# ImIntheMiddle/VATL4Pose-WACV2024

Hardware: AMD Instinct MI355X
Metric: frames/sec pose-infer+uncertainty, 256x192 17-kp (higher is better)
Workload: dtype f32; 1 GPU; SimpleBaseline-R50 256x192 inference + decode + local-peak + THC-L1, 1024-frame synthetic video per GPU; frames_per_gpu=1024, batch=1024, tracks=4, parallelism=frame-sharded x1

## Files before the change

include/vatl_hip.h:

```cpp
#ifndef VATL_HIP_H
#define VATL_HIP_H

#include <stdint.h>

#ifdef __cplusplus
extern "C" {
#endif

#define VATL_VERSION 100
#define VATL_EINVAL  (-1)
#define VATL_ELAUNCH (-2)

int         vatl_version(void);
const char* vatl_last_error(void);

int vatl_flop_meter_begin(void);
int vatl_flop_meter_end(double* direct_flops, double* winograd_flops, int64_t* direct_launches, int64_t* winograd_launches);
#define VATL_ROUTE_NAMES "igemm,igemm_bnbwd,igemm_dma,persistent_1x1,streamk,rows_1x1,bottleneck_chain,stem_pool,halo_3x3," \
                         "winograd,winograd_2h,winograd_bnbwd,winograd_persist,winograd_c32,wgrad,winograd_wgrad,winograd_wgrad_2h," \
                         "winograd_wgrad_table,winograd_f4,winograd_f4_bnbwd,gemm1x1_ring"
int vatl_flop_meter_routes(int64_t* counts, int n);


int vatl_nchw_to_nhwc(const float* src, float* dst, int N, int C, int H, int W, int Cpad, void* stream);
int vatl_nhwc_to_nchw(const float* src, float* dst, int N, int C, int H, int W, void* stream);

int vatl_pack_conv_weight(const float* w_oihw, float* w_packed, int Cout, int Cin, int R, int S,
                          int CoutPad, int Spad, int CinPad, void* stream);
int vatl_pack_deconv4x4s2_weight(const float* w_iohw, float* w_packed, int Cin, int Cout, int CoutPad, void* stream);
int64_t vatl_stem_pool_weight_floats(void);
int vatl_pack_stem_pool_weight(const float* w_oihw, float* packed, void* stream);
int vatl_stem_pool_supported(int H, int W);
int vatl_stem7x7s2_pool_fwd(const float* x_nchw, const float* w_packed, const float* scale, const float* bias, float* y_nhwc,
                            int N, int H, int W, void* stream);
int64_t vatl_stem3_weight_floats(void);
int vatl_pack_stem3_weight(const float* w_oihw, float* packed, void* stream);
int vatl_stem3x3s2_fwd(const float* x_nchw, const float* w_packed, const float* scale, const float* bias, float* y_nhwc,
                       int N, int H, int W, void* stream);

int vatl_bn_fold(const float* gamma, const float* beta, const float* mean, const float* var, const float* conv_bias,
                 float eps, float* scale, float* bias, int C, void* stream);


int vatl_pack_conv1x1_dual_weight(const float* w1, const float* scale1, const float* bias1, const float* w2, const float* scale2,
                                  const float* bias2, float* out, float* bias, int Cout, int C1, int C2, int CoutPad, void* stream);
int vatl_conv1x1_dual_fwd(const float* a, const float* x, const float* w, const float* bias, float* y, int N, int Ho, int Wo,
                          int C1, int H2, int W2, int C2, int stride2, int Cout, int CoutPad, int relu, void* stream);

int64_t vatl_winograd_c32_weight_floats(void);
int vatl_pack_winograd_c32_weight(const float* w, float* u, void* stream);
int vatl_conv3x3_winograd_c32_supported(int N, int H, int W, int Cin, int Cout);
int vatl_conv3x3_winograd_c32_fwd(const float* x, const float* u, const float* scale, const float* bias, const float* residual, float* y, int N, int H, int W,
                                  int relu, void* stream);

int64_t vatl_winograd_f4_weight_floats(int Cout, int Cin);
int vatl_pack_winograd_f4_weight(const float* w, float* u, int Cout, int Cin, int data_gradient, void* stream);
int vatl_conv3x3_winograd_f4_supported(int N, int H, int W, int Cin, int Cout);
int vatl_conv3x3_winograd_f4_fwd(const float* x, const float* u, const float* scale, const float* bias, const float* residual, float* y, int N, int H, int W,
                                 int Cin, int Cout, int relu, void* stream);
int64_t vatl_winograd_f4_stats_row_blocks(int64_t N, int H, int W);
int vatl_conv3x3_winograd_f4_fwd_stats(const float* x, const float* u, float* y, double* stats, int64_t* row_blocks_used, int N, int H, int W, int Cin, int Cout,
                                       void* stream);
int vatl_conv3x3_winograd_f4_fwd_bnbwd(const float* x, const float* u, const float* residual, float* y, int N, int H, int W, int Cin, int Cout, const float* bn_z,
                                       const float* bn_mask_y, const float* bn_scale, const float* bn_bias, const float* bn_mean, const float* bn_invstd,
                                       double* stats, int64_t* row_blocks_used, void* stream);

int vatl_conv1x1_rows_supported(int K1, int K2, int N, int64_t M);
int vatl_conv1x1_rows_fwd(const float* a, const float* x2, const float* w, const float* scale, const float* bias, const float* residual, float* y,
                          int64_t M, int K1, int K2, int N, int relu, void* stream);

int vatl_bottleneck_chain_supported(int Cmid, int Cout, int Cnext, int64_t M);
int vatl_bottleneck_chain_fwd(const float* a, const float* w3, const float* scale3, const float* bias3, const float* skip, float* t,
                              const float* w1, const float* scale1, const float* bias1, float* y1, int64_t M, int Cmid, int Cout,
                              int Cnext, void* stream);

int vatl_tune_set(int knob, int value);
int vatl_set_splitk_workspace(float* workspace, int64_t floats);
int vatl_set_splitk_workspace_thread(float* workspace, int64_t floats);
int64_t vatl_streamk_workspace_bytes(void);
int vatl_set_streamk_workspace_thread(void* workspace, int64_t bytes);
int vatl_conv_cout_pad(int Cout);
int vatl_conv2d_fwd(const float* x, const float* w, const float* scale, const float* bias, const float* residual,
                    float* y, int N, int H, int W, int Cin, int Cout, int CoutPad, int R, int S, int stride, int pad,
                    int relu, int out_nchw, void* stream);

int vatl_deconv4x4s2_fwd(const float* x, const float* w, const float* scale, const float* bias, float* y,
                         int N, int H, int W, int Cin, int Cout, int CoutPad, int relu, void* stream);

int vatl_maxpool3x3s2_fwd(const float* x, float* y, int N, int H, int W, int C, void* stream);
int vatl_gap_fwd(const float* x, float* y, int N, int HW, int C, void* stream);

int vatl_pixelshuffle2_fwd(const float* x, float* y, int N, int H, int W, int C, void* stream);
int vatl_se_scale_add_relu(const float* x, const float* gate, const float* residual, float* y, int N, int HW, int C, void* stream);
int vatl_fuse_upsample_add(const float* base, const float* z0, int shift0, const float* z1, int shift1, const float* z2, int shift2,
                           float* y, int N, int H, int W, int C, int relu, void* stream);
int vatl_upsample_nearest_bwd(const float* dy, const float* yact_or_null, float* dz, int N, int H, int W, int C, int shift, void* stream);
int vatl_gap_bwd(const float* dy, float* dx, int N, int HW, int C, void* stream);


int vatl_decode_argmax_affine(const float* hm, const float* bbox, float* coords, float* maxvals, int32_t* idx,
                              int N, int J, int H, int W, void* stream);
int vatl_decode_pose(const float* hm, const float* bbox, float* kpts, int32_t* idx, float* hp, double* pose_score,
                     int N, int J, int H, int W, void* stream);

int vatl_thc_pairs(const float* a, const float* b, int64_t stride_a, int64_t stride_b, float* out,
                   int P, int J, int HW, int norm, void* stream);
int vatl_thc_combine(const float* pair, const uint8_t* is_prev, const uint8_t* is_next, float* thc, int N, void* stream);

int vatl_localpeak_mean(const float* hm, float* mean, int32_t* count, double* workspace, int N, int J, int H, int W, float order,
                        void* stream);

int vatl_hybrid_ae_wpu(const float* kpts, const float* bbox, const float* ae, int D, int z, int only38,
                       float* wpu, int32_t* status, int N, void* stream);

int vatl_tpc_stream(const float* cur, const float* adj_prev, const float* adj_next, const float* bbox,
                    const uint8_t* is_prev, const uint8_t* is_next, float* tpc, int N, int J, void* stream);

int vatl_decode_softargmax(const float* hm, const float* bbox, float* coords, float* scores,
                           int N, int J, int H, int W, int norm_type, void* stream);

int vatl_ae_forward(const float* feat, const float* ae, int D, int z, float* recon, float* mse, int N, void* stream);

// ... 171 lines not shown
```

vatl4pose-wacv2024_amd/alphapose/models/hip_engine.py:

```python
from __future__ import annotations

import time
import weakref

import torch
import torch.nn as nn

import vatl_hip as vh

MAX_CHUNK = 1024



WINOGRAD = True
ROWS_GEMM = True
ROWS_GEMM_K = (128, 256)
WINO_C32 = True
WINO_F4 = True


class _Conv:
    __slots__ = ("w", "u", "u32", "u4", "wsrc", "wino", "c32", "f4", "scale", "bias", "cout", "r", "s", "stride", "pad")

    def __init__(self, conv: nn.Conv2d, bn: nn.BatchNorm2d | None):
        assert conv.groups == 1 and conv.dilation == (1, 1)
        assert conv.stride[0] == conv.stride[1] and conv.padding[0] == conv.padding[1]
        self.w = vh.pack_conv_weight(conv.weight.detach())
        self.cout, _, self.r, self.s = conv.weight.shape
        self.stride, self.pad = conv.stride[0], conv.padding[0]
        self.u = self.u32 = self.u4 = None
        self.wino = WINOGRAD and (self.r, self.s, self.stride, self.pad) == (3, 3, 1, 1) and conv.in_channels % 16 == 0 and self.cout % 4 == 0
        self.c32 = self.wino and WINO_C32 and conv.in_channels == 32 and self.cout == 32
        self.f4 = self.wino and WINO_F4 and conv.in_channels >= 64 and conv.in_channels % 16 == 0 and self.cout % 64 == 0
        self.wsrc = conv.weight.detach() if self.wino else None
        cb = conv.bias.detach() if conv.bias is not None else None
        if bn is not None:
            self.scale, self.bias = vh.bn_fold(_d(bn.weight), _d(bn.bias), bn.running_mean, bn.running_var, bn.eps, cb)
        elif cb is not None:
            self.scale, self.bias = vh.bn_fold(None, None, None, None, 0.0, cb, channels=self.cout)
        else:
            self.scale = self.bias = None

    def __call__(self, x, relu, residual=None, out_nchw=False, out=None):
        if self.wino and not out_nchw and not vh.latency_mode():
            if self.c32 and vh.conv3x3_winograd_c32_supported(x.shape[0], x.shape[1], x.shape[2], 32, 32):
                if self.u32 is None:
                    self.u32 = vh.pack_winograd_c32_weight(self.wsrc)
                return vh.conv3x3_winograd_c32_fwd(x, self.u32, self.scale, self.bias, relu, residual=residual, out=out)
            if self.f4 and vh.conv3x3_winograd_f4_supported(x.shape[0], x.shape[1], x.shape[2], x.shape[3], self.cout):
                if self.u4 is None:
                    self.u4 = vh.pack_winograd_f4_weight(self.wsrc)
                return vh.conv3x3_winograd_f4_fwd(x, self.u4, self.scale, self.bias, self.cout, relu, residual=residual, out=out)
            if self.u is None:
                self.u = vh.pack_winograd_weight(self.wsrc)
            return vh.conv3x3_winograd_fwd(x, self.u, self.scale, self.bias, self.cout, relu, residual=residual, out=out)
        if (ROWS_GEMM and self.r == 1 and self.stride == 1 and not out_nchw and not vh.latency_mode() and x.shape[-1] in ROWS_GEMM_K
                and vh.conv1x1_rows_supported(x.shape[-1], 0, self.cout, x.shape[0] * x.shape[1] * x.shape[2])):
            return vh.conv1x1_rows_fwd(x, self.w, self.scale, self.bias, self.cout, relu, residual=residual, out=out)
        return vh.conv2d_fwd(x, self.w, self.scale, self.bias, self.cout, self.r, self.s, self.stride, self.pad, relu,
                             residual=residual, out_nchw=out_nchw, out=out)


class _Deconv:
    __slots__ = ("w", "u", "scale", "bias", "cout")

    def __init__(self, dc: nn.ConvTranspose2d, bn: nn.BatchNorm2d):
        assert dc.kernel_size == (4, 4) and dc.stride == (2, 2) and dc.padding == (1, 1) and dc.bias is None
        self.cout = dc.weight.shape[1]
        self.u = None
        if WINOGRAD and dc.weight.shape[0] % 16 == 0 and self.cout % 4 == 0:
            self.u = vh.pack_winograd_deconv_weight(dc.weight.detach())
        self.w = vh.pack_deconv_weight(dc.weight.detach())
        self.scale, self.bias = vh.bn_fold(_d(bn.weight), _d(bn.bias), bn.running_mean, bn.running_var, bn.eps)

    def __call__(self, x, relu=True):
        if self.u is not None and not vh.latency_mode():
            return vh.deconv4x4s2_winograd_fwd(x, self.u, self.scale, self.bias, self.cout, relu)
        return vh.deconv4x4s2_fwd(x, self.w, self.scale, self.bias, self.cout, relu)


def _d(p):
    return None if p is None else p.detach()


FUSE_PROJ = True


class _BottleneckPlan:
    def __init__(self, blk):
        self.c1 = _Conv(blk.conv1, blk.bn1)
        self.c2 = _Conv(blk.conv2, blk.bn2)
        self.c3 = _Conv(blk.conv3, blk.bn3)
        self.proj = _Conv(blk.downsample[0], blk.downsample[1]) if blk.downsample is not None else None
        self.dual = None
        if (FUSE_PROJ and self.proj is not None and type(self) is _BottleneckPlan and self.proj.r == 1 and self.c3.cout >= 128
                and blk.conv3.in_channels % 32 == 0 and blk.downsample[0].in_channels % 32 == 0):
            w, b = vh.pack_conv1x1_dual_weight(blk.conv3.weight.detach(), self.c3.scale, self.c3.bias, blk.downsample[0].weight.detach(),
                                               self.proj.scale, self.proj.bias)
            self.dual = (w, b, self.proj.stride)

    def __call__(self, x, out=None, y1=None):
        y = y1 if y1 is not None else self.c1(x, relu=True)
        y = self.c2(y, relu=True)
        return self.tail(y, x, out=out)

    def tail(self, y, x, out=None):
        if self.dual is not None:
            if (ROWS_GEMM and self.dual[2] == 1 and y.shape[-1] == 64 and x.shape[-1] == 64 and not vh.latency_mode()
                    and vh.conv1x1_rows_supported(64, 64, self.c3.cout, y.shape[0] * y.shape[1] * y.shape[2])):
                return vh.conv1x1_rows_fwd(y, self.dual[0], None, self.dual[1], self.c3.cout, True, x2=x, out=out)
            return vh.conv1x1_dual_fwd(y, x, self.dual[0], self.dual[1], self.c3.cout, self.dual[2], True, out=out)
# ... 458 lines not shown
```

vatl4pose-wacv2024_amd/csrc/common.h:

```cpp
#pragma once
#include <hip/hip_runtime.h>
#include <atomic>
#include <cstdarg>
#include <cstdio>
#include <cstdint>

#include "vatl_hip.h"

namespace vatl {

char* err_buf();
int fail(int code, const char* fmt, ...);

void meter_add(int kind, double flops);
enum MeterRoute {
    kRouteIgemm = 0, kRouteIgemmBnBwd, kRouteIgemmDma, kRoutePersistent1x1, kRouteStreamK, kRouteRows, kRouteChain, kRouteStemPool, kRouteHalo,
    kRouteWino, kRouteWino2H, kRouteWinoBnBwd, kRouteWinoPersist, kRouteWinoC32, kRouteWgrad, kRouteWinoWgrad, kRouteWinoWgrad2H,
    kRouteWinoWgradTable, kRouteWinoF4, kRouteWinoF4BnBwd, kRouteGemm1x1Ring, kRouteCount
};
void meter_route(int route);

inline int check_launch(const char* what) {
    hipError_t e = hipGetLastError();
    if (e != hipSuccess) return fail(VATL_ELAUNCH, "%s: %s", what, hipGetErrorString(e));
    return 0;
}

inline int ensure_dynamic_lds(const void* kern, int bytes, std::atomic<unsigned>& done_mask, const char* what) {
    int d = 0;
    if (hipGetDevice(&d) != hipSuccess) return fail(VATL_ELAUNCH, "%s: no current device", what);
    const unsigned bit = 1u << (d & 31);
    if (done_mask.load(std::memory_order_acquire) & bit) return 0;
    hipError_t e = hipFuncSetAttribute(kern, hipFuncAttributeMaxDynamicSharedMemorySize, bytes);
    if (e != hipSuccess) return fail(VATL_ELAUNCH, "hipFuncSetAttribute(%s): %s", what, hipGetErrorString(e));
    done_mask.fetch_or(bit, std::memory_order_release);
    return 0;
}

__attribute__((visibility("hidden"))) int conv3x3_halo_try(const float* x, const float* w, const float* scale, const float* bias, const float* residual, float* y, int N, int H, int W,
                                                           int Cin, int Cout, int CoutPad, int R, int S, int stride, int pad, int relu, hipStream_t st);

static inline int cdiv(int64_t a, int64_t b) { return (int)((a + b - 1) / b); }

typedef float f32x4 __attribute__((ext_vector_type(4)));
typedef float f32x16 __attribute__((ext_vector_type(16)));

__device__ __forceinline__ void lds_barrier() {
    asm volatile("s_waitcnt lgkmcnt(0)" ::: "memory");
    __builtin_amdgcn_s_barrier();
    asm volatile("" ::: "memory");
}

__device__ __forceinline__ float wave_sum(float v) {
#pragma unroll
    for (int o = 32; o > 0; o >>= 1) v += __shfl_xor(v, o, 64);
    return v;
}
__device__ __forceinline__ double wave_sum(double v) {
#pragma unroll
    for (int o = 32; o > 0; o >>= 1) v += __shfl_xor(v, o, 64);
    return v;
}
__device__ __forceinline__ float wave_max(float v) {
#pragma unroll
    for (int o = 32; o > 0; o >>= 1) v = fmaxf(v, __shfl_xor(v, o, 64));
    return v;
}
__device__ __forceinline__ int wave_sum(int v) {
#pragma unroll
    for (int o = 32; o > 0; o >>= 1) v += __shfl_xor(v, o, 64);
    return v;
// ... 19 lines not shown
```

vatl4pose-wacv2024_amd/vatl_hip/__init__.py:

```python
from __future__ import annotations

import ctypes as C
import os
import threading as _threading

import torch

_HERE = os.path.dirname(os.path.abspath(__file__))
LIB_PATH = os.environ.get("VATL_HIP_LIB") or os.path.join(_HERE, "libvatl_hip.so")

_p = C.c_void_p
_i = C.c_int
_f = C.c_float
_d = C.c_double
_i64 = C.c_int64

SIGNATURES = {
    "vatl_version": (_i, []),
    "vatl_last_error": (C.c_char_p, []),
    "vatl_flop_meter_begin": (_i, []),
    "vatl_flop_meter_end": (_i, [_p, _p, _p, _p]),
    "vatl_flop_meter_routes": (_i, [_p, _i]),
    "vatl_nchw_to_nhwc": (_i, [_p, _p, _i, _i, _i, _i, _i, _p]),
    "vatl_nhwc_to_nchw": (_i, [_p, _p, _i, _i, _i, _i, _p]),
    "vatl_pack_conv_weight": (_i, [_p, _p, _i, _i, _i, _i, _i, _i, _i, _p]),
    "vatl_pack_deconv4x4s2_weight": (_i, [_p, _p, _i, _i, _i, _p]),
    "vatl_pack_conv1x1_dual_weight": (_i, [_p, _p, _p, _p, _p, _p, _p, _p, _i, _i, _i, _i, _p]),
    "vatl_conv1x1_dual_fwd": (_i, [_p, _p, _p, _p, _p, _i, _i, _i, _i, _i, _i, _i, _i, _i, _i, _i, _p]),
    "vatl_winograd_c32_weight_floats": (_i64, []),
    "vatl_pack_winograd_c32_weight": (_i, [_p, _p, _p]),
    "vatl_conv3x3_winograd_c32_supported": (_i, [_i, _i, _i, _i, _i]),
    "vatl_conv3x3_winograd_c32_fwd": (_i, [_p, _p, _p, _p, _p, _p, _i, _i, _i, _i, _p]),
    "vatl_winograd_f4_weight_floats": (_i64, [_i, _i]),
    "vatl_pack_winograd_f4_weight": (_i, [_p, _p, _i, _i, _i, _p]),
    "vatl_winograd_f4_stats_row_blocks": (_i64, [_i64, _i, _i]),
    "vatl_conv3x3_winograd_f4_fwd_stats": (_i, [_p, _p, _p, _p, _p, _i, _i, _i, _i, _i, _p]),
    "vatl_conv3x3_winograd_f4_fwd_bnbwd": (_i, [_p, _p, _p, _p, _i, _i, _i, _i, _i, _p, _p, _p, _p, _p, _p, _p, _p, _p]),
    "vatl_conv3x3_winograd_f4_supported": (_i, [_i, _i, _i, _i, _i]),
    "vatl_conv3x3_winograd_f4_fwd": (_i, [_p, _p, _p, _p, _p, _p, _i, _i, _i, _i, _i, _i, _p]),
    "vatl_conv1x1_rows_supported": (_i, [_i, _i, _i, _i64]),
    "vatl_conv1x1_rows_fwd": (_i, [_p, _p, _p, _p, _p, _p, _p, _i64, _i, _i, _i, _i, _p]),
    "vatl_bottleneck_chain_supported": (_i, [_i, _i, _i, _i64]),
    "vatl_bottleneck_chain_fwd": (_i, [_p, _p, _p, _p, _p, _p, _p, _p, _p, _p, _i64, _i, _i, _i, _p]),
    "vatl_stem_pool_weight_floats": (_i64, []),
    "vatl_pack_stem_pool_weight": (_i, [_p, _p, _p]),
    "vatl_stem_pool_supported": (_i, [_i, _i]),
    "vatl_stem7x7s2_pool_fwd": (_i, [_p, _p, _p, _p, _p, _i, _i, _i, _p]),
    "vatl_stem3_weight_floats": (_i64, []),
    "vatl_pack_stem3_weight": (_i, [_p, _p, _p]),
    "vatl_stem3x3s2_fwd": (_i, [_p, _p, _p, _p, _p, _i, _i, _i, _p]),
    "vatl_bn_fold": (_i, [_p, _p, _p, _p, _p, _f, _p, _p, _i, _p]),
    "vatl_tune_set": (_i, [_i, _i]),
    "vatl_set_splitk_workspace": (_i, [_p, _i64]),
    "vatl_set_splitk_workspace_thread": (_i, [_p, _i64]),
    "vatl_streamk_workspace_bytes": (_i64, []),
    "vatl_set_streamk_workspace_thread": (_i, [_p, _i64]),
    "vatl_conv_cout_pad": (_i, [_i]),
    "vatl_conv2d_fwd": (_i, [_p, _p, _p, _p, _p, _p, _i, _i, _i, _i, _i, _i, _i, _i, _i, _i, _i, _i, _p]),
    "vatl_deconv4x4s2_fwd": (_i, [_p, _p, _p, _p, _p, _i, _i, _i, _i, _i, _i, _i, _p]),
    "vatl_maxpool3x3s2_fwd": (_i, [_p, _p, _i, _i, _i, _i, _p]),
    "vatl_gap_fwd": (_i, [_p, _p, _i, _i, _i, _p]),
    "vatl_pixelshuffle2_fwd": (_i, [_p, _p, _i, _i, _i, _i, _p]),
    "vatl_se_scale_add_relu": (_i, [_p, _p, _p, _p, _i, _i, _i, _p]),
    "vatl_fuse_upsample_add": (_i, [_p, _p, _i, _p, _i, _p, _i, _p, _i, _i, _i, _i, _i, _p]),
    "vatl_upsample_nearest_bwd": (_i, [_p, _p, _p, _i, _i, _i, _i, _i, _p]),
    "vatl_gap_bwd": (_i, [_p, _p, _i, _i, _i, _p]),
    "vatl_decode_argmax_affine": (_i, [_p, _p, _p, _p, _p, _i, _i, _i, _i, _p]),
    "vatl_decode_pose": (_i, [_p, _p, _p, _p, _p, _p, _i, _i, _i, _i, _p]),
    "vatl_thc_pairs": (_i, [_p, _p, _i64, _i64, _p, _i, _i, _i, _i, _p]),
    "vatl_thc_combine": (_i, [_p, _p, _p, _p, _i, _p]),
    "vatl_localpeak_mean": (_i, [_p, _p, _p, _p, _i, _i, _i, _i, _f, _p]),
    "vatl_hybrid_ae_wpu": (_i, [_p, _p, _p, _i, _i, _i, _p, _p, _i, _p]),
    "vatl_tpc_stream": (_i, [_p, _p, _p, _p, _p, _p, _p, _i, _i, _p]),
    "vatl_decode_softargmax": (_i, [_p, _p, _p, _p, _i, _i, _i, _i, _i, _p]),
    "vatl_ae_forward": (_i, [_p, _p, _i, _i, _p, _p, _i, _p]),
    "vatl_hybrid_feature_f64": (_i, [_p, _p, _p, _p, _i, _p]),
    "vatl_localpeak_mask": (_i, [_p, _p, _i, _i, _i, _f, _p]),
    "vatl_peaks5": (_i, [_p, _p, _p, _p, _p, _p, _i, _i, _i, _i, _i, _p]),
    "vatl_plane_entropy": (_i, [_p, _p, _i, _i, _i, _i, _p]),
    "vatl_conv2d_fwd_ex": (_i, [_p] * 6 + [_i] * 20 + [_p]),
    "vatl_conv2d_fwd_ex_bnbwd": (_i, [_p] * 4 + [_i] * 19 + [_p] * 9),
    "vatl_bn_bwd_from_stats": (_i, [_p, _i64, _p, _p, _p, _p, _p, _p, _p, _p, _i64, _i, _p, _p]),
    "vatl_pack_dgrad_weight": (_i, [_p, _p, _i, _i, _i, _i, _i, _i, _i, _p, _p, _p]),
    "vatl_conv2d_wgrad_workspace_floats": (_i64, [_i, _i, _i, _i, _i64]),
    "vatl_conv2d_wgrad": (_i, [_p, _p, _p, _p, _i, _i, _i, _i, _i, _i, _i, _i, _i, _i, _p]),
    "vatl_deconv4x4s2_wgrad_workspace_floats": (_i64, [_i, _i, _i64]),
    "vatl_deconv4x4s2_wgrad": (_i, [_p, _p, _p, _p, _i, _i, _i, _i, _i, _p]),
    "vatl_col_reduce_workspace_doubles": (_i64, [_i64, _i]),
    "vatl_bn_train_fwd_stats": (_i, [_p, _i64, _i, _p, _p, _p, _p, _f, _f, _p, _p, _p, _p, _p, _p]),
    "vatl_scale_bias_act": (_i, [_p, _p, _p, _p, _p, _i64, _i, _i, _p]),
    "vatl_bn_train_bwd": (_i, [_p, _p, _p, _p, _p, _p, _p, _p, _p, _p, _i64, _i, _p, _p, _p]),
    "vatl_bn_train_bwd_relu": (_i, [_p, _p, _p, _p, _p, _p, _p, _p, _p, _p, _i64, _i, _p, _p, _p]),
    "vatl_conv_stats_row_blocks": (_i64, [_i64, _i]),
    "vatl_winograd_cout_pad": (_i, [_i]),
# ... 90 lines not shown
    t = torch.as_tensor(host)
    device = torch.device(device)
    if t.is_cuda:
        return t.to(device=device, dtype=dtype if dtype is not None else t.dtype)
    if dtype is not None and t.dtype != dtype:
        t = t.to(dtype)
    if device.type != "cuda" or t.numel() == 0:
        return t.to(device)
    if owned and t.is_pinned() and t.is_contiguous():
        return t.to(device, non_blocking=True)
    stage = torch.empty(t.shape, dtype=t.dtype, pin_memory=True)
    stage.copy_(t)
    return stage.to(device, non_blocking=True)


def _ptr(t, dtype=torch.float32):
    if t is None:
        return None
    if not t.is_cuda:
        raise VatlError("vatl_hip needs device (HIP) tensors; there is no CPU path")
    if t.dtype != dtype:
        raise VatlError(f"expected {dtype}, got {t.dtype}")
    if not t.is_contiguous():
        raise VatlError("tensor must be contiguous")
    return t.data_ptr()


def _stream():
    return torch.cuda.current_stream().cuda_stream


_tls = _threading.local()



def nchw_to_nhwc(x: torch.Tensor, cpad: int | None = None) -> torch.Tensor:
    n, c, h, w = x.shape
    cpad = cpad or c
    y = torch.empty((n, h, w, cpad), device=x.device, dtype=torch.float32)
    _check(lib().vatl_nchw_to_nhwc(_ptr(x), _ptr(y), n, c, h, w, cpad, _stream()), "vatl_nchw_to_nhwc")
    return y


def nhwc_to_nchw(x: torch.Tensor) -> torch.Tensor:
    n, h, w, c = x.shape
    y = torch.empty((n, c, h, w), device=x.device, dtype=torch.float32)
    _check(lib().vatl_nhwc_to_nchw(_ptr(x), _ptr(y), n, c, h, w, _stream()), "vatl_nhwc_to_nchw")
    return y



ROUTE_NAMES = ("igemm", "igemm_bnbwd", "igemm_dma", "persistent_1x1", "streamk", "rows_1x1", "bottleneck_chain", "stem_pool", "halo_3x3", "winograd",
               "winograd_2h", "winograd_bnbwd", "winograd_persist", "winograd_c32", "wgrad", "winograd_wgrad", "winograd_wgrad_2h", "winograd_wgrad_table", "winograd_f4", "winograd_f4_bnbwd",
               "gemm1x1_ring")


class flop_meter:

    def __enter__(self):
        _check(lib().vatl_flop_meter_begin(), "flop_meter_begin")
        self.direct = self.winograd = self.total = 0.0
        self.direct_launches = self.winograd_launches = 0
        return self

    @staticmethod
    def launches_now() -> int:
        counts = (C.c_int64 * len(ROUTE_NAMES))()
        _check(min(0, lib().vatl_flop_meter_routes(counts, len(ROUTE_NAMES))), "flop_meter_routes")
        return int(sum(counts))

    def __exit__(self, *exc):
        counts = (C.c_int64 * len(ROUTE_NAMES))()
        _check(min(0, lib().vatl_flop_meter_routes(counts, len(ROUTE_NAMES))), "flop_meter_routes")
        self.routes = {n: int(c) for n, c in zip(ROUTE_NAMES, counts)}
        d, w, nd, nw = C.c_double(0), C.c_double(0), C.c_int64(0), C.c_int64(0)
        _check(lib().vatl_flop_meter_end(C.byref(d), C.byref(w), C.byref(nd), C.byref(nw)), "flop_meter_end")
        self.direct, self.winograd, self.total = d.value, w.value, d.value + w.value
        self.direct_launches, self.winograd_launches = nd.value, nw.value
        return False


def tune_set(knob: int, value: int):
    _check(lib().vatl_tune_set(knob, value), "vatl_tune_set")


_splitk_buf = {}


def enable_splitk(megabytes: int = 64, device=None):
    dev = torch.device(device) if device is not None else torch.device("cuda", torch.cuda.current_device())
    idx = dev.index if dev.index is not None else torch.cuda.current_device()
    with torch.cuda.device(idx):
        if megabytes <= 0:
            _check(lib().vatl_set_splitk_workspace(None, 0), "vatl_set_splitk_workspace")
            _splitk_buf.pop(idx, None)
            return
        buf = torch.empty(megabytes * (1 << 18), device=torch.device("cuda", idx), dtype=torch.float32)
        _check(lib().vatl_set_splitk_workspace(_ptr(buf), buf.numel()), "vatl_set_splitk_workspace")
        _splitk_buf[idx] = buf


_splitk_scratch = {}
_splitk_scratch_lock = _threading.Lock()
SPLITK_SCRATCH_MB = 256


class splitk_scope:
# ... 257 lines not shown
    _check(lib().vatl_pack_winograd_c32_weight(_ptr(w.contiguous()), _ptr(out), _stream()), "vatl_pack_winograd_c32_weight")
    return out


def pack_stem_pool_weight(w: torch.Tensor) -> torch.Tensor:
    if tuple(w.shape) != (64, 3, 7, 7):
        raise VatlError(f"pack_stem_pool_weight: expected a (64,3,7,7) filter, got {tuple(w.shape)}")
    w = w.detach().float().contiguous()
    out = torch.empty(int(lib().vatl_stem_pool_weight_floats()), device=w.device, dtype=torch.float32)
    _check(lib().vatl_pack_stem_pool_weight(_ptr(w), _ptr(out), _stream()), "vatl_pack_stem_pool_weight")
    return out


def pack_stem3_weight(w: torch.Tensor) -> torch.Tensor:
    if tuple(w.shape) != (64, 3, 3, 3):
        raise VatlError(f"pack_stem3_weight: expected a (64,3,3,3) filter, got {tuple(w.shape)}")
    w = w.detach().float().contiguous()
    out = torch.empty(int(lib().vatl_stem3_weight_floats()), device=w.device, dtype=torch.float32)
    _check(lib().vatl_pack_stem3_weight(_ptr(w), _ptr(out), _stream()), "vatl_pack_stem3_weight")
    return out


def bn_fold(gamma, beta, mean, var, eps: float, conv_bias=None, channels: int | None = None):
    c = channels if channels is not None else (var.numel() if var is not None else conv_bias.numel())
    dev = (var if var is not None else conv_bias).device
    scale = torch.empty(c, device=dev, dtype=torch.float32)
    bias = torch.empty(c, device=dev, dtype=torch.float32)
    _check(lib().vatl_bn_fold(_ptr(gamma), _ptr(beta), _ptr(mean), _ptr(var), _ptr(conv_bias), eps, _ptr(scale), _ptr(bias), c, _stream()), "vatl_bn_fold")
    return scale, bias



def conv2d_fwd(x, w_packed, scale, bias, cout: int, r: int, s: int, stride: int, pad: int, relu: bool,
               residual=None, out_nchw: bool = False, out=None):
    n, h, w, cin = x.shape
    ho = (h + 2 * pad - r) // stride + 1
    wo = (w + 2 * pad - s) // stride + 1
    shape = (n, cout, ho, wo) if out_nchw else (n, ho, wo, cout)
    y = out if out is not None else torch.empty(shape, device=x.device, dtype=torch.float32)
    _check(lib().vatl_conv2d_fwd(_ptr(x), _ptr(w_packed), _ptr(scale), _ptr(bias), _ptr(residual), _ptr(y), n, h, w, cin, cout,
                                 w_packed.shape[0], r, s, stride, pad, int(relu), int(out_nchw), _stream()), "vatl_conv2d_fwd")
    return y


def conv1x1_dual_fwd(a, x, w_packed, bias, cout: int, stride2: int, relu: bool, out=None):
    n, ho, wo, c1 = a.shape
    _, h2, w2, c2 = x.shape
    y = out if out is not None else torch.empty((n, ho, wo, cout), device=a.device, dtype=torch.float32)
    _check(lib().vatl_conv1x1_dual_fwd(_ptr(a), _ptr(x), _ptr(w_packed), _ptr(bias), _ptr(y), n, ho, wo, c1, h2, w2, c2, stride2, cout,
                                       w_packed.shape[0], int(relu), _stream()), "vatl_conv1x1_dual_fwd")
    return y


def conv1x1_rows_supported(k1: int, k2: int, n: int, m: int) -> bool:
    return bool(lib().vatl_conv1x1_rows_supported(k1, k2, n, m))


def conv1x1_rows_fwd(a, w, scale, bias, cout: int, relu: bool, residual=None, x2=None, out=None):
    n, h, w_, k1 = a.shape
    k2 = 0 if x2 is None else x2.shape[-1]
    assert w.numel() >= cout * (k1 + k2) and (x2 is None or tuple(x2.shape[:3]) == (n, h, w_)) and (residual is None or tuple(residual.shape) == (n, h, w_, cout))
    y = out if out is not None else torch.empty((n, h, w_, cout), device=a.device, dtype=torch.float32)
    assert a.is_contiguous() and y.is_contiguous() and (x2 is None or x2.is_contiguous()) and (residual is None or residual.is_contiguous())
    _check(lib().vatl_conv1x1_rows_fwd(_ptr(a), _ptr(x2), _ptr(w), _ptr(scale), _ptr(bias), _ptr(residual), _ptr(y), n * h * w_, k1, k2, cout, int(relu),
                                       _stream()), "vatl_conv1x1_rows_fwd")
    return y


def bottleneck_chain_supported(cmid: int, cout: int, cnext: int, m: int) -> bool:
    return bool(lib().vatl_bottleneck_chain_supported(cmid, cout, cnext, m))


def bottleneck_chain_fwd(a, w3, scale3, bias3, skip, w1=None, scale1=None, bias1=None, out=None, y1_out=None):
    n, h, w_, cmid = a.shape
    cout = w3.shape[0]
    cnext = 0 if w1 is None else w1.shape[0]
    assert w3.numel() == cout * cmid and (w1 is None or w1.numel() == cnext * cout) and (skip is None or tuple(skip.shape) == (n, h, w_, cout))
    t = out if out is not None else torch.empty((n, h, w_, cout), device=a.device, dtype=torch.float32)
    assert t.is_contiguous() and a.is_contiguous() and (skip is None or skip.is_contiguous())
    y1 = None if w1 is None else (y1_out if y1_out is not None else torch.empty((n, h, w_, cnext), device=a.device, dtype=torch.float32))
    _check(lib().vatl_bottleneck_chain_fwd(_ptr(a), _ptr(w3), _ptr(scale3), _ptr(bias3), _ptr(skip), _ptr(t), _ptr(w1), _ptr(scale1), _ptr(bias1), _ptr(y1),
                                           n * h * w_, cmid, cout, cnext, _stream()), "vatl_bottleneck_chain_fwd")
    return t, y1


def stem3_fwd(x_nchw: torch.Tensor, w_packed: torch.Tensor, scale: torch.Tensor, bias: torch.Tensor) -> torch.Tensor:
    n, c, h, w = x_nchw.shape
    if c != 3:
        raise VatlError(f"stem3_fwd: expected 3 input channels, got {c}")
    y = torch.empty((n, h // 2, w // 2, 64), device=x_nchw.device, dtype=torch.float32)
    _check(lib().vatl_stem3x3s2_fwd(_ptr(x_nchw), _ptr(w_packed), _ptr(scale), _ptr(bias), _ptr(y), n, h, w, _stream()), "vatl_stem3x3s2_fwd")
    return y


def stem_pool_supported(h: int, w: int) -> bool:
    return bool(lib().vatl_stem_pool_supported(int(h), int(w)))


def stem_pool_fwd(x_nchw: torch.Tensor, w_packed: torch.Tensor, scale: torch.Tensor, bias: torch.Tensor, out=None) -> torch.Tensor:
    n, c, h, w = x_nchw.shape
    if c != 3:
        raise VatlError(f"stem_pool_fwd: expected 3 input channels, got {c}")
    y = out if out is not None else torch.empty((n, h // 4, w // 4, 64), device=x_nchw.device, dtype=torch.float32)
    _check(lib().vatl_stem7x7s2_pool_fwd(_ptr(x_nchw), _ptr(w_packed), _ptr(scale), _ptr(bias), _ptr(y), n, h, w, _stream()), "vatl_stem7x7s2_pool_fwd")
    return y


def conv3x3_winograd_fwd(x, u_packed, scale, bias, cout: int, relu: bool, residual=None, out=None):
    n, h, w, cin = x.shape
    y = out if out is not None else torch.empty((n, h, w, cout), device=x.device, dtype=torch.float32)
    _check(lib().vatl_conv3x3_winograd_fwd(_ptr(x), _ptr(u_packed), _ptr(scale), _ptr(bias), _ptr(residual), _ptr(y), n, h, w, cin, cout,
                                           int(relu), _stream()), "vatl_conv3x3_winograd_fwd")
    return y
# ... 792 lines not shown
```

Before: 16490 frames/s.

## Add narrow-N MFMA 1x1 conv kernel for 64-channel and head convs

Adds a persistent 1x1 convolution kernel for narrow outputs (N=64 NHWC with K=64/256, and K=256 with N<=32 writing NCHW planes for the heatmap head). It keeps the weights in registers, streams activation tiles into LDS with buffer-to-LDS loads and double buffering, and uses fp32 MFMA 32x32x2. The Python routing sends cout<=64 pointwise convs to it instead of the generic implicit GEMM. The intent is to cut the padding waste and poor utilisation of the generic path on narrow-N GEMMs, in exchange for added code complexity and a persistent-grid schedule that depends on residency.

```diff
diff --git a/include/vatl_hip.h b/include/vatl_hip.h
--- a/include/vatl_hip.h
+++ b/include/vatl_hip.h
@@ -18,7 +18,7 @@
 int vatl_flop_meter_end(double* direct_flops, double* winograd_flops, int64_t* direct_launches, int64_t* winograd_launches);
 #define VATL_ROUTE_NAMES "igemm,igemm_bnbwd,igemm_dma,persistent_1x1,streamk,rows_1x1,bottleneck_chain,stem_pool,halo_3x3," \
                          "winograd,winograd_2h,winograd_bnbwd,winograd_persist,winograd_c32,wgrad,winograd_wgrad,winograd_wgrad_2h," \
-                         "winograd_wgrad_table,winograd_f4,winograd_f4_bnbwd,gemm1x1_ring"
+                         "winograd_wgrad_table,winograd_f4,winograd_f4_bnbwd,gemm1x1_ring,narrow_1x1"
 int vatl_flop_meter_routes(int64_t* counts, int n);
 
 
@@ -68,6 +68,10 @@
 int vatl_conv1x1_rows_supported(int K1, int K2, int N, int64_t M);
 int vatl_conv1x1_rows_fwd(const float* a, const float* x2, const float* w, const float* scale, const float* bias, const float* residual, float* y,
                           int64_t M, int K1, int K2, int N, int relu, void* stream);
+
+int vatl_conv1x1_narrow_supported(int K, int N, int64_t M, int out_nchw);
+int vatl_conv1x1_narrow_fwd(const float* a, const float* w, const float* scale, const float* bias, const float* residual, float* y, int64_t M, int HW,
+                            int K, int N, int relu, int out_nchw, void* stream);
 
 int vatl_bottleneck_chain_supported(int Cmid, int Cout, int Cnext, int64_t M);
 int vatl_bottleneck_chain_fwd(const float* a, const float* w3, const float* scale3, const float* bias3, const float* skip, float* t,
diff --git a/vatl4pose-wacv2024_amd/alphapose/models/hip_engine.py b/vatl4pose-wacv2024_amd/alphapose/models/hip_engine.py
--- a/vatl4pose-wacv2024_amd/alphapose/models/hip_engine.py
+++ b/vatl4pose-wacv2024_amd/alphapose/models/hip_engine.py
@@ -15,6 +15,7 @@
 WINOGRAD = True
 ROWS_GEMM = True
 ROWS_GEMM_K = (128, 256)
+NARROW_GEMM = True
 WINO_C32 = True
 WINO_F4 = True
 
@@ -54,9 +55,12 @@
             if self.u is None:
                 self.u = vh.pack_winograd_weight(self.wsrc)
             return vh.conv3x3_winograd_fwd(x, self.u, self.scale, self.bias, self.cout, relu, residual=residual, out=out)
-        if (ROWS_GEMM and self.r == 1 and self.stride == 1 and not out_nchw and not vh.latency_mode() and x.shape[-1] in ROWS_GEMM_K
+        if (ROWS_GEMM and self.r == 1 and self.stride == 1 and self.cout >= 128 and not out_nchw and not vh.latency_mode() and x.shape[-1] in ROWS_GEMM_K
                 and vh.conv1x1_rows_supported(x.shape[-1], 0, self.cout, x.shape[0] * x.shape[1] * x.shape[2])):
             return vh.conv1x1_rows_fwd(x, self.w, self.scale, self.bias, self.cout, relu, residual=residual, out=out)
+        if (NARROW_GEMM and self.r == 1 and self.stride == 1 and self.pad == 0 and self.cout <= 64 and not vh.latency_mode() and (residual is None or not out_nchw)
+                and vh.conv1x1_rows_supported(x.shape[-1], 0, self.cout, x.shape[0] * x.shape[1] * x.shape[2], out_nchw=out_nchw)):
+            return vh.conv1x1_rows_fwd(x, self.w, self.scale, self.bias, self.cout, relu, residual=residual, out=out, out_nchw=out_nchw)
         return vh.conv2d_fwd(x, self.w, self.scale, self.bias, self.cout, self.r, self.s, self.stride, self.pad, relu,
                              residual=residual, out_nchw=out_nchw, out=out)
 
diff --git a/vatl4pose-wacv2024_amd/csrc/common.h b/vatl4pose-wacv2024_amd/csrc/common.h
--- a/vatl4pose-wacv2024_amd/csrc/common.h
+++ b/vatl4pose-wacv2024_amd/csrc/common.h
@@ -16,7 +16,7 @@
 enum MeterRoute {
     kRouteIgemm = 0, kRouteIgemmBnBwd, kRouteIgemmDma, kRoutePersistent1x1, kRouteStreamK, kRouteRows, kRouteChain, kRouteStemPool, kRouteHalo,
     kRouteWino, kRouteWino2H, kRouteWinoBnBwd, kRouteWinoPersist, kRouteWinoC32, kRouteWgrad, kRouteWinoWgrad, kRouteWinoWgrad2H,
-    kRouteWinoWgradTable, kRouteWinoF4, kRouteWinoF4BnBwd, kRouteGemm1x1Ring, kRouteCount
+    kRouteWinoWgradTable, kRouteWinoF4, kRouteWinoF4BnBwd, kRouteGemm1x1Ring, kRouteNarrow1x1, kRouteCount
 };
 void meter_route(int route);
 
diff --git a/vatl4pose-wacv2024_amd/csrc/conv1x1_narrow.hip b/vatl4pose-wacv2024_amd/csrc/conv1x1_narrow.hip
--- /dev/null
+++ b/vatl4pose-wacv2024_amd/csrc/conv1x1_narrow.hip
@@ -0,0 +1,182 @@
+#include "common.h"
+#include "buffer.h"
+
+#ifndef NARROW_ALT
+#define NARROW_ALT 0
+#endif
+
+namespace vatl {
+
+struct NarrowParams {
+    const float* a;
+    const float* w;
+    const float* scale;
+    const float* bias;
+    const float* res;
+    float* y;
+    int M, N, relu, m_tiles, HW;
+    FastDivU d_hw;
+    unsigned a_bytes, y_bytes, w_bytes;
+};
+
+constexpr unsigned NR_OOB = 0xFFFFFFFFu;
+
+__device__ __forceinline__ unsigned narrow_stage_base(int mt, int m_tiles, int tile_bytes, int kc_bytes) {
+    return (unsigned)(mt < m_tiles ? mt : m_tiles) * (unsigned)tile_bytes + (unsigned)kc_bytes;
+}
+
+template <int K, int KC, bool HEAD, bool RES>
+__global__ __launch_bounds__(128, (K == 64 ? 4 : 2)) void conv1x1_narrow_kernel(NarrowParams p) {
+    constexpr int TP = HEAD ? 64 : 32;
+    constexpr int NKC = K / KC;
+    constexpr int CPR = KC / 4;
+    constexpr int STG = TP * KC;
+    constexpr int U = TP * CPR / 128;
+    constexpr int GC = KC / 8;
+    static_assert(K % KC == 0 && (NKC == 1 || NKC % 2 == 0) && KC % 32 == 0 && U >= 1, "stage geometry");
+    extern __shared__ __attribute__((aligned(16))) float smem[];
+    float* As = smem;
+    const int tid = threadIdx.x, lane = tid & 63, wave = __builtin_amdgcn_readfirstlane(tid >> 6);
+    const int fr = lane & 31, h = lane >> 5;
+    const int nblk = gridDim.x;
+    const int pg = HEAD ? wave : 0;
+    const int nw = (HEAD ? 0 : wave * 32) + fr;
+
+    const __amdgpu_buffer_rsrc_t ar = buf_rsrc(p.a, p.a_bytes);
+    const __amdgpu_buffer_rsrc_t wr = buf_rsrc(p.w, p.w_bytes);
+    const __amdgpu_buffer_rsrc_t yr = buf_rsrc(p.y, p.y_bytes);
+    const __amdgpu_buffer_rsrc_t rr = buf_rsrc(RES ? p.res : p.y, RES ? p.y_bytes : 0u);
+
+    f32x4 wf[K / 8];
+#pragma unroll
+    for (int g = 0; g < K / 8; ++g) wf[g] = buf_load4(wr, (unsigned)((nw * K + 8 * g + 4 * h) * 4));
+    constexpr int NS = HEAD ? 16 : 1;
+    float sc[NS], bi[NS];
+#pragma unroll
+    for (int e = 0; e < NS; ++e) {
+        const int n = HEAD ? (e & 3) + 8 * (e >> 2) + 4 * h : nw;
+        const bool nv = n < p.N;
+        sc[e] = (nv && p.scale) ? p.scale[n] : 1.f;
+        bi[e] = (nv && p.bias) ? p.bias[n] : 0.f;
+    }
+    const float lo = p.relu ? 0.f : -INFINITY;
+
+    unsigned lanev[U];
+#pragma unroll
+    for (int u = 0; u < U; ++u) {
+        const int q = (wave * U + u) * 64 + lane;
+        const int row = q / CPR, chunk = (q % CPR) ^ (row & 7);
+        lanev[u] = (unsigned)(row * K + chunk * 4) * 4u;
+    }
+    const unsigned nrow = (unsigned)p.N * 4u;
+    const unsigned ylane = (unsigned)((4 * h) * p.N + nw) * 4u;
+    const unsigned hw4 = (unsigned)p.HW * 4u;
+    int mt = blockIdx.x, buf = 0;
+    {
+        const unsigned base = narrow_stage_base(mt, p.m_tiles, TP * K * 4, 0);
+#pragma unroll
+        for (int u = 0; u < U; ++u) {
+            const unsigned off = base + lanev[u];
+            __builtin_amdgcn_raw_ptr_buffer_load_lds(ar, (lds_void*)(As + (wave * U + u) * 256), 16, off, 0, 0, 0);
+        }
+    }
+    asm volatile("s_waitcnt vmcnt(0)" ::: "memory");
+    for (; mt < p.m_tiles; mt += nblk) {
+        const unsigned ybase = (unsigned)mt * (32u * nrow) + ylane;
+        float rs[16];
+        f32x16 acc;
+#pragma unroll
+        for (int kc = 0; kc < NKC; ++kc) {
+            const int stage = NKC == 1 ? buf : (kc & 1);
+            if (kc == 0) asm volatile("s_waitcnt vmcnt(16)" ::: "memory");
+            else asm volatile("s_waitcnt vmcnt(0)" ::: "memory");
+            lds_barrier();
+            if (kc == 0) {
+#pragma unroll
+                for (int e = 0; e < 16; ++e) rs[e] = RES ? buf_load1(rr, ybase + (unsigned)((e & 3) + 8 * (e >> 2)) * nrow) : 0.f;
+            }
+            {
+                const unsigned base = kc + 1 < NKC ? narrow_stage_base(mt, p.m_tiles, TP * K * 4, (kc + 1) * KC * 4) : narrow_stage_base(mt + nblk, p.m_tiles, TP * K * 4, 0);
+#pragma unroll
+                for (int u = 0; u < U; ++u) {
+                    const unsigned off = base + lanev[u];
+                    __builtin_amdgcn_raw_ptr_buffer_load_lds(ar, (lds_void*)(As + (stage ^ 1) * STG + (wave * U + u) * 256), 16, off, 0, 0, 0);
+                }
+            }
+            __builtin_amdgcn_sched_barrier(0);
+            const float* at = As + stage * STG + (pg * 32 + fr) * KC;
+#pragma unroll
+            for (int gl = 0; gl < GC; ++gl) {
+                const int g = kc * GC + gl;
+                const f32x4 af = *reinterpret_cast<const f32x4*>(at + (((2 * gl + h) ^ (fr & 7)) << 2));
+#pragma unroll
+                for (int tt = 0; tt < 4; ++tt) {
+                    const f32x16 c = (g == 0 && tt == 0) ? f32x16{0.f, 0.f, 0.f, 0.f, 0.f, 0.f, 0.f, 0.f, 0.f, 0.f, 0.f, 0.f, 0.f, 0.f, 0.f, 0.f} : acc;
+                    if constexpr (HEAD) acc = __builtin_amdgcn_mfma_f32_32x32x2f32(wf[g][tt], af[tt], c, 0, 0, 0);
+                    else acc = __builtin_amdgcn_mfma_f32_32x32x2f32(af[tt], wf[g][tt], c, 0, 0, 0);
+                }
+            }
+        }
+        if constexpr (NKC == 1) buf ^= 1;
+        if constexpr (HEAD) {
+            const int m = mt * 64 + pg * 32 + fr;
+            const int b = fdiv(m, p.d_hw);
+            const unsigned pbase = ((unsigned)(b * p.N + 4 * h) * (unsigned)p.HW + (unsigned)(m - b * p.HW)) * 4u;
+            const bool mv = m < p.M;
+#pragma unroll
+            for (int e = 0; e < 16; ++e) {
+                const int ce = (e & 3) + 8 * (e >> 2);
+                const unsigned off = (mv && ce + 4 * h < p.N) ? pbase + (unsigned)ce * hw4 : NR_OOB;
+                buf_store1(yr, off, fmaxf(acc[e] * sc[e] + bi[e], lo));
+            }
+        } else {
+#pragma unroll
+            for (int e = 0; e < 16; ++e) buf_store1(yr, ybase + (unsigned)((e & 3) + 8 * (e >> 2)) * nrow, fmaxf(acc[e] * sc[0] + bi[0] + rs[e], lo));
+        }
+    }
+}
+
+}
+
+using namespace vatl;
+
+static bool narrow_shape_ok(int K, int N, long long M, int out_nchw) {
+    const bool shape = out_nchw ? (K == 256 && N >= 1 && N <= 32) : ((K == 64 || K == 256) && N == 64);
+    return shape && M > 0 && (M + 64) * (long long)K < (1LL << 30);
+}
+
+extern "C" int vatl_conv1x1_narrow_supported(int K, int N, int64_t M, int out_nchw) { return narrow_shape_ok(K, N, M, out_nchw) ? 1 : 0; }
+
+static int narrow_launch(void (*kern)(NarrowParams), int smem, std::atomic<unsigned>& configured, const NarrowParams& p, int blocks_per_cu, hipStream_t st) {
+    if (int rc = ensure_dynamic_lds(reinterpret_cast<const void*>(kern), smem, configured, "conv1x1_narrow")) return rc;
+    const int resident = 256 * blocks_per_cu;
+    const int grid = p.m_tiles < resident ? p.m_tiles : resident;
+    hipLaunchKernelGGL(kern, dim3(grid), dim3(128), smem, st, p);
+    return 0;
+}
+
+extern "C" int vatl_conv1x1_narrow_fwd(const float* a, const float* w, const float* scale, const float* bias, const float* residual, float* y, int64_t M, int HW,
+                                       int K, int N, int relu, int out_nchw, void* stream) {
+    if (!a || !w || !y || (out_nchw && (residual || HW <= 0 || M % HW != 0))) return fail(VATL_EINVAL, "conv1x1_narrow_fwd: bad arguments");
+    if (!narrow_shape_ok(K, N, M, out_nchw))
+        return fail(VATL_EINVAL, "conv1x1_narrow_fwd: serves K = 64 / 256 with N = 64 (NHWC) and K = 256 with N <= 32 (NCHW planes), (M + 64) * K < 2^30");
+    const int tp = out_nchw ? 64 : 32, npad = (N + 31) / 32 * 32;
+    NarrowParams p{};
+    p.a = a; p.w = w; p.scale = scale; p.bias = bias; p.res = residual; p.y = y;
+    p.M = (int)M; p.N = N; p.relu = relu; p.m_tiles = (int)((M + tp - 1) / tp); p.HW = out_nchw ? HW : 1;
+    p.d_hw = make_fastdiv((unsigned)p.HW);
+    p.a_bytes = (unsigned)(M * K * 4); p.y_bytes = (unsigned)(M * N * 4); p.w_bytes = (unsigned)(npad * K * 4);
+    const hipStream_t st = (hipStream_t)stream;
+    static std::atomic<unsigned> c0{0}, c1{0}, c2{0}, c3{0}, c4{0};
+    constexpr int KCH = NARROW_ALT ? 128 : 64, KCN = NARROW_ALT ? 256 : 128, BPC = NARROW_ALT ? 2 : 4;
+    int rc;
+    if (out_nchw) rc = narrow_launch(conv1x1_narrow_kernel<256, KCH, true, false>, 2 * 64 * KCH * 4, c0, p, BPC, st);
+    else if (K == 64 && residual) rc = narrow_launch(conv1x1_narrow_kernel<64, 64, false, true>, 2 * 32 * 64 * 4, c1, p, 2 * BPC, st);
+    else if (K == 64) rc = narrow_launch(conv1x1_narrow_kernel<64, 64, false, false>, 2 * 32 * 64 * 4, c2, p, 2 * BPC, st);
+    else if (residual) rc = narrow_launch(conv1x1_narrow_kernel<256, KCN, false, true>, 2 * 32 * KCN * 4, c3, p, BPC, st);
+    else rc = narrow_launch(conv1x1_narrow_kernel<256, KCN, false, false>, 2 * 32 * KCN * 4, c4, p, BPC, st);
+    if (rc) return rc;
+    meter_add(0, 2.0 * ((double)p.m_tiles * tp) * (double)npad * (double)K);
+    meter_route(kRouteNarrow1x1);
+    return check_launch("conv1x1_narrow");
+}
diff --git a/vatl4pose-wacv2024_amd/vatl_hip/__init__.py b/vatl4pose-wacv2024_amd/vatl_hip/__init__.py
--- a/vatl4pose-wacv2024_amd/vatl_hip/__init__.py
+++ b/vatl4pose-wacv2024_amd/vatl_hip/__init__.py
@@ -40,6 +40,8 @@
     "vatl_conv3x3_winograd_f4_fwd": (_i, [_p, _p, _p, _p, _p, _p, _i, _i, _i, _i, _i, _i, _p]),
     "vatl_conv1x1_rows_supported": (_i, [_i, _i, _i, _i64]),
     "vatl_conv1x1_rows_fwd": (_i, [_p, _p, _p, _p, _p, _p, _p, _i64, _i, _i, _i, _i, _p]),
+    "vatl_conv1x1_narrow_supported": (_i, [_i, _i, _i64, _i]),
+    "vatl_conv1x1_narrow_fwd": (_i, [_p, _p, _p, _p, _p, _p, _i64, _i, _i, _i, _i, _i, _p]),
     "vatl_bottleneck_chain_supported": (_i, [_i, _i, _i, _i64]),
     "vatl_bottleneck_chain_fwd": (_i, [_p, _p, _p, _p, _p, _p, _p, _p, _p, _p, _i64, _i, _i, _i, _p]),
     "vatl_stem_pool_weight_floats": (_i64, []),
@@ -236,7 +238,7 @@
 
 ROUTE_NAMES = ("igemm", "igemm_bnbwd", "igemm_dma", "persistent_1x1", "streamk", "rows_1x1", "bottleneck_chain", "stem_pool", "halo_3x3", "winograd",
                "winograd_2h", "winograd_bnbwd", "winograd_persist", "winograd_c32", "wgrad", "winograd_wgrad", "winograd_wgrad_2h", "winograd_wgrad_table", "winograd_f4", "winograd_f4_bnbwd",
-               "gemm1x1_ring")
+               "gemm1x1_ring", "narrow_1x1")
 
 
 class flop_meter:
@@ -600,13 +602,26 @@
     return y
 
 
-def conv1x1_rows_supported(k1: int, k2: int, n: int, m: int) -> bool:
-    return bool(lib().vatl_conv1x1_rows_supported(k1, k2, n, m))
-
-
-def conv1x1_rows_fwd(a, w, scale, bias, cout: int, relu: bool, residual=None, x2=None, out=None):
+def conv1x1_rows_supported(k1: int, k2: int, n: int, m: int, out_nchw: bool = False) -> bool:
+    if n <= 64:
+        return k2 == 0 and bool(lib().vatl_conv1x1_narrow_supported(k1, n, m, int(out_nchw)))
+    return not out_nchw and bool(lib().vatl_conv1x1_rows_supported(k1, k2, n, m))
+
+
+def conv1x1_rows_fwd(a, w, scale, bias, cout: int, relu: bool, residual=None, x2=None, out=None, out_nchw: bool = False):
     n, h, w_, k1 = a.shape
     k2 = 0 if x2 is None else x2.shape[-1]
+    if cout <= 64:
+        if x2 is not None or (out_nchw and residual is not None):
+            raise VatlError("conv1x1_rows_fwd: the narrow kernel takes one source and no residual with NCHW output")
+        assert w.numel() >= (cout + 31) // 32 * 32 * k1 and (residual is None or tuple(residual.shape) == (n, h, w_, cout))
+        y = out if out is not None else torch.empty((n, cout, h, w_) if out_nchw else (n, h, w_, cout), device=a.device, dtype=torch.float32)
+        assert a.is_contiguous() and y.is_contiguous() and y.numel() == n * h * w_ * cout and (residual is None or residual.is_contiguous())
+        _check(lib().vatl_conv1x1_narrow_fwd(_ptr(a), _ptr(w), _ptr(scale), _ptr(bias), _ptr(residual), _ptr(y), n * h * w_, h * w_, k1, cout, int(relu),
+                                             int(out_nchw), _stream()), "vatl_conv1x1_narrow_fwd")
+        return y
+    if out_nchw:
+        raise VatlError("conv1x1_rows_fwd: NCHW output is served for cout <= 32 only")
     assert w.numel() >= cout * (k1 + k2) and (x2 is None or tuple(x2.shape[:3]) == (n, h, w_)) and (residual is None or tuple(residual.shape) == (n, h, w_, cout))
     y = out if out is not None else torch.empty((n, h, w_, cout), device=a.device, dtype=torch.float32)
     assert a.is_contiguous() and y.is_contiguous() and (x2 is None or x2.is_contiguous()) and (residual is None or residual.is_contiguous())
```

Measured after the change: 16560 frames/s (median of 6 runs). About the same (+0.5%).
